# mobvoi/lstm_ctc

Measured on AMD Instinct MI355X. Metric: acoustic frames/sec (whole node), 5xBiLSTM-1024 CTC, higher is better.
Workload: dtype f32

## Files before the change

### lstm_ctc_amd/csrc/common.h

```cpp
#pragma once
#include <hip/hip_runtime.h>
#include <stdint.h>
#include <stdio.h>
#include <stdarg.h>
#include "../../include/lstm_ctc_hip.h"

#define LC_WAVE 64

void lc_set_error(const char *fmt, ...);
enum { LC_OPT_LSTM_PERSISTENT = 0, LC_OPT_LSTM_SPIN_LIMIT, LC_OPT_GEMM_F32_BIG, LC_OPT_GEMM_BF16_BIG, LC_OPT_CTC_LSE2,
       LC_OPT_GEMM_BF16_PERSIST, LC_OPT_GEMM_TAIL };
long lc_option(int opt, long dflt);

#define LC_CHECK_ARG(cond, ...)                                   \
    do {                                                          \
        if (!(cond)) { lc_set_error(__VA_ARGS__); return LC_EINVAL; } \
    } while (0)

#define LC_CHECK_LAUNCH(what)                                                        \
    do {                                                                             \
        hipError_t e_ = hipGetLastError();                                           \
        if (e_ != hipSuccess) {                                                      \
            lc_set_error("%s: %s", what, hipGetErrorString(e_));                     \
            return LC_ELAUNCH;                                                       \
        }                                                                            \
    } while (0)

static inline int lc_cdiv(long long a, long long b) { return (int)((a + b - 1) / b); }

__host__ __device__ inline uint32_t lc_fmix32(uint32_t h)
{
    h ^= h >> 16; h *= 0x85EBCA6Bu; h ^= h >> 13; h *= 0xC2B2AE35u; h ^= h >> 16;
    return h;
}
__host__ __device__ inline float lc_dropout_factor(uint32_t seed, uint32_t stream, uint64_t idx,
                                                   float keep, float inv_keep)
{
    uint32_t h = (seed * 0x9E3779B1u) ^ (stream * 0x85EBCA77u + 0x165667B1u);
    uint32_t v = lc_fmix32((uint32_t)idx ^ h);
    v = lc_fmix32(v ^ ((uint32_t)(idx >> 32) + 0x27D4EB2Fu));
    float u = (float)(v >> 8) * (1.0f / 16777216.0f);
    return u < keep ? inv_keep : 0.0f;
}

__device__ __forceinline__ float lc_wave_shr1(float x, float fill)
{
    return __int_as_float(__builtin_amdgcn_update_dpp(__float_as_int(fill), __float_as_int(x),
                                                      0x138, 0xf, 0xf, false));
}
__device__ __forceinline__ float lc_wave_shl1(float x, float fill)
{
    return __int_as_float(__builtin_amdgcn_update_dpp(__float_as_int(fill), __float_as_int(x),
                                                      0x130, 0xf, 0xf, false));
}
#define LC_DPP_STEP(OP, v, ctrl, rowmask)                                                                   \
    v = OP(v, __int_as_float(__builtin_amdgcn_update_dpp(__float_as_int(v), __float_as_int(v), ctrl, rowmask, \
                                                         0xf, false)))
__device__ __forceinline__ float lc_addf(float a, float b) { return a + b; }
__device__ __forceinline__ float lc_wave_max(float v)
{
    LC_DPP_STEP(fmaxf, v, 0x111, 0xf);
    LC_DPP_STEP(fmaxf, v, 0x112, 0xf);
    LC_DPP_STEP(fmaxf, v, 0x114, 0xf);
    LC_DPP_STEP(fmaxf, v, 0x118, 0xf);
    LC_DPP_STEP(fmaxf, v, 0x142, 0xa);
    LC_DPP_STEP(fmaxf, v, 0x143, 0xc);
    return __int_as_float(__builtin_amdgcn_readlane(__float_as_int(v), 63));
}
__device__ __forceinline__ float lc_wave_sum(float v)
{
#define LC_DPP_ADD(ctrl, rowmask)                                                                            \
    v += __int_as_float(__builtin_amdgcn_update_dpp(0, __float_as_int(v), ctrl, rowmask, 0xf, true))
    LC_DPP_ADD(0x111, 0xf);
    LC_DPP_ADD(0x112, 0xf);
    LC_DPP_ADD(0x114, 0xf);
    LC_DPP_ADD(0x118, 0xf);
    LC_DPP_ADD(0x142, 0xa);
    LC_DPP_ADD(0x143, 0xc);
#undef LC_DPP_ADD
    return __int_as_float(__builtin_amdgcn_readlane(__float_as_int(v), 63));
}
__device__ __forceinline__ float lc_sigmoid(float x)
{
    return __builtin_amdgcn_rcpf(1.0f + __builtin_amdgcn_exp2f(-1.44269504088896341f * x));
}
__device__ __forceinline__ float lc_tanh(float x)
{
    const float t = __builtin_amdgcn_exp2f(-2.88539008177792681f * fabsf(x));
    return copysignf((1.0f - t) * __builtin_amdgcn_rcpf(1.0f + t), x);
}
```

### lstm_ctc_amd/csrc/error.cpp

```cpp
#include <limits.h>
#include <stdarg.h>
#include <stdio.h>
#include <stdlib.h>
#include <string.h>
#include "../../include/lstm_ctc_hip.h"

static thread_local char g_err[512] = "";

void lc_set_error(const char *fmt, ...)
{
    va_list ap;
    va_start(ap, fmt);
    vsnprintf(g_err, sizeof(g_err), fmt, ap);
    va_end(ap);
}

extern "C" const char *lc_last_error(void) { return g_err; }
extern "C" int lc_version(void) { return 2; }

static const char *const g_opt_name[] = {"lstm_persistent", "lstm_spin_limit", "gemm_f32_big", "gemm_bf16_big", "ctc_lse2",
                                         "gemm_bf16_persist", "gemm_tail"};
static const char *const g_opt_env[] = {"LC_LSTM_PERSISTENT", "LC_LSTM_SPIN_LIMIT", "LC_GEMM_F32_BIG",
                                        "LC_GEMM_BF16_BIG", "LC_CTC_LSE2", "LC_GEMM_BF16_PERSIST",
                                        "LC_GEMM_TAIL"};
enum { N_OPTS = sizeof(g_opt_name) / sizeof(g_opt_name[0]) };
static thread_local long g_opt_val[N_OPTS];
static thread_local bool g_opt_set[N_OPTS];

long lc_option(int opt, long dflt)
{
    if (opt < 0 || opt >= N_OPTS) return dflt;
    if (g_opt_set[opt]) return g_opt_val[opt];
    const char *env = getenv(g_opt_env[opt]);
    return env ? atol(env) : dflt;
}
static int opt_index(const char *name)
{
    for (int i = 0; name && i < N_OPTS; ++i)
        if (strcmp(name, g_opt_name[i]) == 0) return i;
    return -1;
}
extern "C" int lc_set_option(const char *name, long value)
{
    const int i = opt_index(name);
    if (i < 0) { lc_set_error("lc_set_option: unknown option '%s'", name ? name : "(null)"); return LC_EINVAL; }
    g_opt_set[i] = value != LC_OPTION_UNSET;
    g_opt_val[i] = value;
    return LC_OK;
}
extern "C" int lc_get_option(const char *name, long *value)
{
    const int i = opt_index(name);
    if (i < 0) { lc_set_error("lc_get_option: unknown option '%s'", name ? name : "(null)"); return LC_EINVAL; }
    const long v = lc_option(i, LC_OPTION_UNSET);
    if (value) *value = v;
    return LC_OK;
}
```

### lstm_ctc_amd/csrc/gemm.hip

```cpp
#include "common.h"
#include "gemm_epi.h"
#include <algorithm>

typedef float f32x16 __attribute__((ext_vector_type(16)));
typedef int i32x4 __attribute__((ext_vector_type(4)));
typedef float f32x4v __attribute__((ext_vector_type(4)));
__device__ f32x4v lc_raw_buffer_load_f32x4(i32x4 rsrc, int voffset, int soffset, int aux) __asm("llvm.amdgcn.raw.buffer.load.v4f32");
__device__ i32x4 lc_raw_buffer_load_i32x4(i32x4 rsrc, int voffset, int soffset, int aux) __asm("llvm.amdgcn.raw.buffer.load.v4i32");

namespace {

#ifndef LC_GEMM_BK
#define LC_GEMM_BK 16
#endif
#ifndef LC_GEMM_GROUP_M
#define LC_GEMM_GROUP_M 8
#endif
constexpr int BM = 128, BN = 128, BK = LC_GEMM_BK, NT = 256;

template <bool KMAJOR, bool FAST, int I>
__device__ __forceinline__ float4 tile_load1(const float *__restrict__ src, int ld, int c0, int cmax, int k0,
                                             int kmax, bool vec_ok)
{
    const int f = threadIdx.x + NT * I;
// ... 705 lines not shown
#pragma unroll
    for (int q = 0; q < 4; ++q) maa[q] = lds0 + arow + so[q];
#define LC_MLOAD(Q, FA, FB)                                                                                            \
    {                                                                                                                  \
        lds_read128<0>(maa[Q] + tbuf, FA[0]); lds_read128<4096>(maa[Q] + tbuf, FA[1]);                                 \
        lds_read128<8192>(maa[Q] + tbuf, FA[2]); lds_read128<12288>(maa[Q] + tbuf, FA[3]);                             \
        _Pragma("unroll") for (int j = 0; j < 2; ++j) tr16_pair<(Q) * 8192>(tob[j] + tbuf, FB[j][0], FB[j][1]);        \
    }
#define LC_MWAIT(FA, FB)                                                                                               \
    asm volatile("s_waitcnt lgkmcnt(0)"                                                                                \
                 : "+v"(FA[0]), "+v"(FA[1]), "+v"(FA[2]), "+v"(FA[3]), "+v"(FB[0][0]), "+v"(FB[0][1]), "+v"(FB[1][0]),  \
                   "+v"(FB[1][1]));
#define LC_MMMA(FA, FB)                                                                                                \
    _Pragma("unroll") for (int i = 0; i < 4; ++i)                                                                      \
        _Pragma("unroll") for (int j = 0; j < 2; ++j)                                                                  \
            acc[i][j] = __builtin_amdgcn_mfma_f32_32x32x16_bf16(frag_cast(FA[i]), tr16_join(FB[j][0], FB[j][1]),        \
                                                               acc[i][j], 0, 0, 0);
#define LC_MCOMPUTE(BUF)                                                                                               \
    {                                                                                                                  \
        const unsigned tbuf = (BUF) * 2 * G_OPERAND_BYTES;                                                             \
        i32x4g m0a[4], m1a[4];                                                                                         \
        i32x2 m0b[2][2], m1b[2][2];                                                                                    \
        LC_MLOAD(0, m0a, m0b) LC_MWAIT(m0a, m0b)                                                                       \
        LC_MLOAD(1, m1a, m1b) LC_MMMA(m0a, m0b) LC_MWAIT(m1a, m1b)                                                     \
        LC_MLOAD(2, m0a, m0b) LC_MMMA(m1a, m1b) LC_MWAIT(m0a, m0b)                                                     \
        LC_MLOAD(3, m1a, m1b) LC_MMMA(m0a, m0b) LC_MWAIT(m1a, m1b)                                                     \
        LC_MMMA(m1a, m1b)                                                                                              \
    }
#define LC_GCOMPUTE(BUF)                                                                                               \
    {                                                                                                                  \
        const unsigned char *as = lds + (BUF) * 2 * G_OPERAND_BYTES;                                                   \
        const unsigned char *bs = lds + ((BUF) * 2 + 1) * G_OPERAND_BYTES;                                             \
        bf16x8 a[4], b[2];                                                                                             \
        _Pragma("unroll") for (int i = 0; i < 4; ++i) a[i] = LC_GFRAG_A(i, 0);                                         \
        _Pragma("unroll") for (int j = 0; j < 2; ++j) b[j] = LC_GFRAG_B(j, 0);                                         \
        _Pragma("unroll") for (int q = 0; q < 4; ++q) {                                                                \
            bf16x8 na[4], nb[2];                                                                                       \
            if (q + 1 < 4) {                                                                                           \
                _Pragma("unroll") for (int i = 0; i < 4; ++i) na[i] = LC_GFRAG_A(i, (q + 1) & 3);                      \
                _Pragma("unroll") for (int j = 0; j < 2; ++j) nb[j] = LC_GFRAG_B(j, (q + 1) & 3);                      \
            }                                                                                                          \
            _Pragma("unroll") for (int i = 0; i < 4; ++i)                                                              \
                _Pragma("unroll") for (int j = 0; j < 2; ++j)                                                          \
                    acc[i][j] = __builtin_amdgcn_mfma_f32_32x32x16_bf16(a[i], b[j], acc[i][j], 0, 0, 0);               \
            if (q + 1 < 4) {                                                                                           \
                _Pragma("unroll") for (int i = 0; i < 4; ++i) a[i] = na[i];                                            \
                _Pragma("unroll") for (int j = 0; j < 2; ++j) b[j] = nb[j];                                            \
            }                                                                                                          \
        }                                                                                                              \
    }
#define LC_GSYNC()                                                                                                     \
    {                                                                                                                  \
        if constexpr (ACOL || BCOL) asm volatile("s_waitcnt vmcnt(0)" ::: "memory");                                   \
        __syncthreads();                                                                                               \
    }
#define LC_GDO(BUF)                                                                                                    \
    {                                                                                                                  \
        if constexpr (ACOL) LC_TCOMPUTE(BUF) else if constexpr (BCOL) LC_MCOMPUTE(BUF) else LC_GCOMPUTE(BUF)            \
    }
    const int ntiles = (p.M / GBM) * (p.N / GBN);
    LC_GFILL(0, 0)
    LC_GSYNC()
    for (int vb = blockIdx.x;;) {
#pragma unroll
    for (int i = 0; i < 4; ++i)
#pragma unroll
        for (int j = 0; j < 2; ++j)
#pragma unroll
            for (int r = 0; r < 16; ++r) acc[i][j][r] = 0.f;
    int nm0 = m0, nn0 = n0;
    bool more = false;
    __amdgpu_buffer_rsrc_t ra_n = ra, rb_n = rb;
    if constexpr (PERSIST) {
        const int vn = vb + (int)gridDim.x;
        more = vn < ntiles;
        if (more) {
            int bm_, bn_;
            gemm_tile_order_big(p.M, p.N, bm_, bn_, vn);
            nm0 = bm_ * GBM; nn0 = bn_ * GBN;
            ra_n = rsrc_a(nm0); rb_n = rsrc_b(nn0);
        }
    }
    int kt = 0;
    for (; kt + 2 <= nk; kt += 2) {
        LC_GFILL(min(kt + 1, nk - 1), 1)
        LC_GDO(0)
        LC_GSYNC()
        if (PERSIST && kt + 2 >= nk) {
            LC_GFILL_FROM(ra_n, rb_n, 0, 0)
        } else {
            LC_GFILL(min(kt + 2, nk - 1), 0)
        }
        LC_GDO(1)
        LC_GSYNC()
    }
    if (kt < nk) LC_GDO(0)
#undef LC_GCOMPUTE
#undef LC_GFRAG
#undef LC_GFRAG_A
#undef LC_GFRAG_B
#undef LC_TLOAD
#undef LC_TWAIT
#undef LC_TMMA
#undef LC_TCOMPUTE
#undef LC_MLOAD
#undef LC_MWAIT
#undef LC_MMMA
#undef LC_MCOMPUTE
    if (p.slab) {
        float *S = p.slab + (size_t)blockIdx.z * p.slab_slice;
#pragma unroll
        for (int i = 0; i < 4; ++i)
#pragma unroll
            for (int j = 0; j < 2; ++j) {
                const int col = n0 + wn * 64 + j * 32 + lr;
#pragma unroll
                for (int r = 0; r < 16; ++r) {
                    const int row = m0 + wm * 128 + i * 32 + (r & 3) + 8 * (r >> 2) + 4 * lk;
                    S[(size_t)row * p.slab_ld + col] = acc[i][j][r];
                }
            }
        return;
    }
#pragma unroll
    for (int i = 0; i < 4; ++i)
#pragma unroll
        for (int j = 0; j < 2; ++j) {
            const int col = n0 + wn * 64 + j * 32 + lr;
            const float bv = p.bias ? p.bias[col] : 0.f;
            unsigned est;
            int ecm;
            epi_column(p.epi, col, est, ecm);
#pragma unroll
            for (int r = 0; r < 16; ++r) {
                const int row = m0 + wm * 128 + i * 32 + (r & 3) + 8 * (r >> 2) + 4 * lk;
                float *c = p.C + (size_t)row * p.ldc + col;
                float v = p.alpha * acc[i][j][r] + bv;
                if (p.beta != 0.f) v += p.beta * *c;
                epi_store(p.epi, c, v, row, col, est, ecm);
            }
        }
    if constexpr (!PERSIST) break;
    if (!more) break;
    vb += (int)gridDim.x;
    m0 = nm0; n0 = nn0; ra = ra_n; rb = rb_n;
    }
#undef LC_GSYNC
#undef LC_GDO
#undef LC_GFILL
#undef LC_GFILL_FROM
}

constexpr int FGBK = 32;
template <bool ACOL, bool BCOL, bool SEG2 = false>
__global__ __launch_bounds__(GNT, 1) void gemm_f32g_kernel(GemmArgs p)
{
    static_assert(!SEG2 || (!ACOL && !BCOL), "two operand pairs: NT form");
    __shared__ __attribute__((aligned(1024))) unsigned char lds[4 * 256 * FGBK * 4];
    constexpr int OPB = 256 * FGBK * 4;
    int bm, bn;
    gemm_tile_order_big(p.M, p.N, bm, bn);
    const int m0 = bm * GBM, n0 = bn * GBN;
    const int lane = threadIdx.x & 63, wave = __builtin_amdgcn_readfirstlane(threadIdx.x >> 6);
    const int wm = wave >> 2, wn = wave & 3;
    const int kbeg = blockIdx.z * p.kchunk;
    const int kend = min(p.K, kbeg + p.kchunk);
    const int nk = (kend - kbeg) / FGBK;
    const float *abase = ACOL ? p.A + (size_t)kbeg * p.lda + m0 : p.A + (size_t)m0 * p.lda + kbeg;
    const float *bbase = BCOL ? p.B + (size_t)kbeg * p.ldb + n0 : p.B + (size_t)n0 * p.ldb + kbeg;
    const __amdgpu_buffer_rsrc_t ra = __builtin_amdgcn_make_buffer_rsrc((void *)abase, 0, 0x7fffffff, 0x00020000);
    const __amdgpu_buffer_rsrc_t rb = __builtin_amdgcn_make_buffer_rsrc((void *)bbase, 0, 0x7fffffff, 0x00020000);
    const int nk1 = SEG2 ? p.k1 / FGBK : nk;
    const __amdgpu_buffer_rsrc_t ra2 = SEG2 ? __builtin_amdgcn_make_buffer_rsrc((void *)(p.A2 + (size_t)m0 * p.lda), 0,
                                                                                0x7fffffff, 0x00020000) : ra;
    const __amdgpu_buffer_rsrc_t rb2 = SEG2 ? __builtin_amdgcn_make_buffer_rsrc((void *)(p.B2 + (size_t)n0 * p.ldb), 0,
                                                                                0x7fffffff, 0x00020000) : rb;
    int voa[4], vob[4];
#pragma unroll
    for (int i = 0; i < 4; ++i) {
        const int piece = wave * 4 + i;
        if (ACOL) voa[i] = (piece * p.lda + 4 * lane) * 4;
        else { const int row = piece * 8 + (lane >> 3); voa[i] = (row * p.lda + ((lane & 7) ^ ((row >> 1) & 7)) * 4) * 4; }
        if (BCOL) vob[i] = (piece * p.ldb + 4 * lane) * 4;
        else { const int row = piece * 8 + (lane >> 3); vob[i] = (row * p.ldb + ((lane & 7) ^ ((row >> 1) & 7)) * 4) * 4; }
    }
    const int ka = ACOL ? FGBK * p.lda * 4 : FGBK * 4, kb = BCOL ? FGBK * p.ldb * 4 : FGBK * 4;
#define LC_FFILL_FROM(RA, RB, KT, BUF)                                                                                 \
    {                                                                                                                  \
        _Pragma("unroll") for (int i = 0; i < 4; ++i)                                                                  \
            __builtin_amdgcn_raw_ptr_buffer_load_lds(RA, lds + (BUF) * 2 * OPB + (wave * 4 + i) * 1024, 16, voa[i],     \
                                                     (KT) * ka, 0, 0);                                                 \
        _Pragma("unroll") for (int i = 0; i < 4; ++i)                                                                  \
            __builtin_amdgcn_raw_ptr_buffer_load_lds(RB, lds + ((BUF) * 2 + 1) * OPB + (wave * 4 + i) * 1024, 16,       \
                                                     vob[i], (KT) * kb, 0, 0);                                         \
    }
#define LC_FFILL(KT, BUF)                                                                                              \
    {                                                                                                                  \
        const int kt_ = (KT);                                                                                          \
        if (SEG2 && kt_ >= nk1) LC_FFILL_FROM(ra2, rb2, kt_ - nk1, BUF) else LC_FFILL_FROM(ra, rb, kt_, BUF)           \
    }
    f32x16 acc[4][2];
#pragma unroll
    for (int i = 0; i < 4; ++i)
#pragma unroll
        for (int j = 0; j < 2; ++j)
#pragma unroll
            for (int r = 0; r < 16; ++r) acc[i][j][r] = 0.f;
    const int lr = lane & 31, lk = lane >> 5;
    const int fl = (lr >> 1) & 7;
    int soq[4];
#pragma unroll
    for (int q = 0; q < 4; ++q) soq[q] = ((2 * q + lk) ^ fl) * 16;
    const int arow = ACOL ? (4 * lk * 256 + wm * 128 + lr) * 4 : (wm * 128 + lr) * 128;
    const int brow = BCOL ? (4 * lk * 256 + wn * 64 + lr) * 4 : (wn * 64 + lr) * 128;
#define LC_FCOMPUTE(BUF)                                                                                               \
    {                                                                                                                  \
        const unsigned char *as = lds + (BUF) * 2 * OPB + arow;                                                        \
        const unsigned char *bs = lds + ((BUF) * 2 + 1) * OPB + brow;                                                  \
        _Pragma("unroll") for (int q = 0; q < 4; ++q) {                                                                \
            float a[4][4], b[2][4];                                                                                    \
            _Pragma("unroll") for (int i = 0; i < 4; ++i) {                                                            \
                if (ACOL) {                                                                                            \
                    _Pragma("unroll") for (int t = 0; t < 4; ++t)                                                      \
                        a[i][t] = *reinterpret_cast<const float *>(as + ((8 * q + t) * 256 + i * 32) * 4);             \
                } else {                                                                                               \
                    const f32x4v v = *reinterpret_cast<const f32x4v *>(as + i * 4096 + soq[q]);                        \
                    a[i][0] = v.x; a[i][1] = v.y; a[i][2] = v.z; a[i][3] = v.w;                                        \
                }                                                                                                      \
            }                                                                                                          \
            _Pragma("unroll") for (int j = 0; j < 2; ++j) {                                                            \
                if (BCOL) {                                                                                            \
                    _Pragma("unroll") for (int t = 0; t < 4; ++t)                                                      \
                        b[j][t] = *reinterpret_cast<const float *>(bs + ((8 * q + t) * 256 + j * 32) * 4);             \
                } else {                                                                                               \
                    const f32x4v v = *reinterpret_cast<const f32x4v *>(bs + j * 4096 + soq[q]);                        \
                    b[j][0] = v.x; b[j][1] = v.y; b[j][2] = v.z; b[j][3] = v.w;                                        \
                }                                                                                                      \
            }                                                                                                          \
            _Pragma("unroll") for (int t = 0; t < 4; ++t)                                                              \
                _Pragma("unroll") for (int i = 0; i < 4; ++i)                                                          \
                    _Pragma("unroll") for (int j = 0; j < 2; ++j)                                                      \
                        acc[i][j] = __builtin_amdgcn_mfma_f32_32x32x2f32(a[i][t], b[j][t], acc[i][j], 0, 0, 0);        \
        }                                                                                                              \
    }
    LC_FFILL(0, 0)
    __syncthreads();
    int kt = 0;
    for (; kt + 2 <= nk; kt += 2) {
        LC_FFILL(min(kt + 1, nk - 1), 1)
        LC_FCOMPUTE(0)
        __syncthreads();
        LC_FFILL(min(kt + 2, nk - 1), 0)
        LC_FCOMPUTE(1)
        __syncthreads();
    }
    if (kt < nk) LC_FCOMPUTE(0)
#undef LC_FFILL
#undef LC_FFILL_FROM
#undef LC_FCOMPUTE
    if (p.slab) {
        float *S = p.slab + (size_t)blockIdx.z * p.slab_slice;
#pragma unroll
        for (int i = 0; i < 4; ++i)
#pragma unroll
            for (int j = 0; j < 2; ++j) {
                const int col = n0 + wn * 64 + j * 32 + lr;
#pragma unroll
                for (int r = 0; r < 16; ++r) {
                    const int row = m0 + wm * 128 + i * 32 + (r & 3) + 8 * (r >> 2) + 4 * lk;
                    S[(size_t)row * p.slab_ld + col] = acc[i][j][r];
                }
            }
        return;
    }
#pragma unroll
    for (int i = 0; i < 4; ++i)
#pragma unroll
        for (int j = 0; j < 2; ++j) {
            const int col = n0 + wn * 64 + j * 32 + lr;
            const float bv = p.bias ? p.bias[col] : 0.f;
            unsigned est;
            int ecm;
            epi_column(p.epi, col, est, ecm);
#pragma unroll
            for (int r = 0; r < 16; ++r) {
                const int row = m0 + wm * 128 + i * 32 + (r & 3) + 8 * (r >> 2) + 4 * lk;
                float *c = p.C + (size_t)row * p.ldc + col;
                float v = p.alpha * acc[i][j][r] + bv;
                if (p.beta != 0.f) v += p.beta * *c;
                epi_store(p.epi, c, v, row, col, est, ecm);
            }
        }
}

__global__ __launch_bounds__(256) void cast_bf16_kernel(const float *__restrict__ x, int rows, int C, int ldx,
                                                        unsigned short *__restrict__ nat, int ldnat,
                                                        unsigned short *__restrict__ tr, int ldtr)
{
    __shared__ unsigned short tile[64][66];
    const int r0 = blockIdx.y * 64, c0 = blockIdx.x * 64;
    const int tx = threadIdx.x & 63, ty = threadIdx.x >> 6;
    for (int i = ty; i < 64; i += 4) {
        const int r = r0 + i, c = c0 + tx;
        unsigned short v = 0;
        if (r < rows && c < C) {
            v = __builtin_bit_cast(unsigned short, (__bf16)x[(size_t)r * ldx + c]);
            if (nat) nat[(size_t)r * ldnat + c] = v;
        }
        tile[i][tx] = v;
    }
    if (!tr) return;
    __syncthreads();
    for (int i = ty; i < 64; i += 4) {
        const int c = c0 + i, r = r0 + tx;
        if (c < C && r < rows) tr[(size_t)c * ldtr + r] = tile[tx][i];
    }
}

__device__ __forceinline__ unsigned cast_pack2(float lo, float hi)
{
    return (unsigned)__builtin_bit_cast(unsigned short, (__bf16)lo) |
           ((unsigned)__builtin_bit_cast(unsigned short, (__bf16)hi) << 16);
}
template <bool NAT, bool TR>
__global__ __launch_bounds__(256) void cast_bf16_vec_kernel(const float *__restrict__ x, int ldx,
                                                            unsigned short *__restrict__ nat, int ldnat,
                                                            unsigned short *__restrict__ tr, int ldtr)
{
    __shared__ __attribute__((aligned(16))) unsigned tile[64 * 32];
    const int r0 = blockIdx.y * 64, c0 = blockIdx.x * 64;
    const int cq = threadIdx.x & 15, rp = threadIdx.x >> 4;
#pragma unroll
    for (int i = 0; i < 2; ++i) {
        const int rpair = rp + 16 * i;
        const size_t r = (size_t)r0 + 2 * rpair;
        const int c = c0 + 4 * cq;
        const float4 v0 = *reinterpret_cast<const float4 *>(x + r * ldx + c);
        const float4 v1 = *reinterpret_cast<const float4 *>(x + (r + 1) * ldx + c);
        if constexpr (NAT) {
            *reinterpret_cast<uint2 *>(nat + r * ldnat + c) = make_uint2(cast_pack2(v0.x, v0.y), cast_pack2(v0.z, v0.w));
            *reinterpret_cast<uint2 *>(nat + (r + 1) * ldnat + c) = make_uint2(cast_pack2(v1.x, v1.y), cast_pack2(v1.z, v1.w));
        }
        if constexpr (TR) {
            const int slot = rpair ^ ((cq & 7) << 2);
            tile[(4 * cq + 0) * 32 + slot] = cast_pack2(v0.x, v1.x);
            tile[(4 * cq + 1) * 32 + slot] = cast_pack2(v0.y, v1.y);
            tile[(4 * cq + 2) * 32 + slot] = cast_pack2(v0.z, v1.z);
            tile[(4 * cq + 3) * 32 + slot] = cast_pack2(v0.w, v1.w);
        }
    }
    if constexpr (TR) {
        __syncthreads();
#pragma unroll
        for (int i = 0; i < 2; ++i) {
            const int c = (threadIdx.x >> 3) + 32 * i, g = threadIdx.x & 7;
            const uint4 v = *reinterpret_cast<const uint4 *>(&tile[c * 32 + ((4 * g) ^ (((c >> 2) & 7) << 2))]);
            *reinterpret_cast<uint4 *>(tr + (size_t)(c0 + c) * ldtr + r0 + 8 * g) = v;
        }
    }
}

__global__ __launch_bounds__(256) void splitk_reduce_kernel(const float *__restrict__ slab, int nslices, int M, int N,
                                                            float alpha, float beta, float *__restrict__ C, int ldc,
                                                            const float *__restrict__ bias)
{
    const size_t total = (size_t)M * N / 4;
    for (size_t i = blockIdx.x * (size_t)blockDim.x + threadIdx.x; i < total; i += (size_t)gridDim.x * blockDim.x) {
        const size_t e = i * 4;
        const int row = (int)(e / N), col = (int)(e % N);
        float4 s = *reinterpret_cast<const float4 *>(slab + e);
        for (int k = 1; k < nslices; ++k) {
            const float4 t = *reinterpret_cast<const float4 *>(slab + (size_t)k * M * N + e);
            s.x += t.x; s.y += t.y; s.z += t.z; s.w += t.w;
        }
        float *c = C + (size_t)row * ldc + col;
        float o[4] = {alpha * s.x, alpha * s.y, alpha * s.z, alpha * s.w};
#pragma unroll
        for (int q = 0; q < 4; ++q) {
            if (bias) o[q] += bias[col + q];
            if (beta != 0.f) o[q] += beta * c[q];
            c[q] = o[q];
        }
    }
}

inline bool aligned16(const void *p) { return (((uintptr_t)p) & 15) == 0; }

inline int pick_splitk(int M, int N, int K)
{
    const long long tiles = (long long)lc_cdiv(M, BM) * lc_cdiv(N, BN);
    if (tiles >= 1536 || K < 4096 || (N % 4) != 0) return 1;
    const long long slots = 768;
    int best = 1;
    double best_eff = 0.0;
    for (int s = 1; s <= 32 && (long long)K / s >= 1024; ++s) {
        const long long wg = tiles * s, rounds = (wg + slots - 1) / slots;
        const double eff = (double)wg / (double)(rounds * slots);
        if (eff > best_eff + 1e-9) { best_eff = eff; best = s; }
    }
    return best;
}

inline int pick_splitk_big(int M, int N, int K, int bk = GBK)
{
    if (M <= 0 || N <= 0 || M % GBM || N % GBN || K < bk || K % bk) return 0;
    const long long tiles = (long long)(M / GBM) * (N / GBN);
    if (tiles >= 512 || K < 4096) return 1;
    int best = 1;
    double best_eff = 0.0;
    for (int c = 1; c <= 32 && K / c >= 1024; ++c) {
        const long long wg = tiles * c, rounds = (wg + 255) / 256;
        const double eff = (double)wg / (double)(rounds * 256);
        if (eff > best_eff + 1e-9) { best_eff = eff; best = c; }
    }
    return best;
}

}

static int lc_num_cus()
{
    static int cached[16] = {0};
    int dev = 0;
    if (hipGetDevice(&dev) != hipSuccess || dev < 0 || dev >= 16) return 256;
    if (cached[dev] == 0) {
        int n = 0;
        if (hipDeviceGetAttribute(&n, hipDeviceAttributeMultiprocessorCount, dev) != hipSuccess || n <= 0) n = 256;
        cached[dev] = n;
    }
    return cached[dev];
}
static int gemm_whole_round_row_tiles(int row_tiles, int col_tiles, int cus_override = 0)
{
    const int cus = cus_override > 0 ? cus_override : lc_num_cus();
    if (lc_option(LC_OPT_GEMM_TAIL, 0) == 0 || row_tiles <= 1 || col_tiles <= 0) return row_tiles;
    const long long tiles = (long long)row_tiles * col_tiles;
    if (tiles % cus == 0 || tiles < 2ll * cus) return row_tiles;
    double best_t = (double)((tiles + cus - 1) / cus) - 0.05;
    int best = row_tiles;
    for (int keep = row_tiles - 1, it = 0; keep >= 1 && it < 512; --keep, ++it) {
        const long long big = (long long)keep * col_tiles, rem = big % cus;
        if (big < cus) break;
        if (rem != 0 && rem * 100 < (long long)cus * 97) continue;
        const double t = (double)((big + cus - 1) / cus) + (double)(row_tiles - keep) * col_tiles * 4 * 0.275 / cus + 0.1;
        if (t < best_t) { best_t = t; best = keep; }
    }
    return best;
}
extern "C" int lc_debug_gemm_whole_round_row_tiles(int row_tiles, int col_tiles, int cus)
{
    return gemm_whole_round_row_tiles(row_tiles, col_tiles, cus);
}
static bool bf16g_persist_ok(long long tiles, int nsl, int K)
{
    const int cus = lc_num_cus();
    return lc_option(LC_OPT_GEMM_BF16_PERSIST, 0) != 0 && nsl <= 1 && K % (2 * GBK) == 0 && cus % 8 == 0 && tiles > cus;
}

static const EpiArgs EPI_NONE = {1.f, 1.f, 0u, 0u, 1, nullptr, 0, 0, 0};
static thread_local EpiArgs g_epi_next = EPI_NONE;
EpiArgs lc_epi_take()
{
    const EpiArgs e = g_epi_next;
    g_epi_next = EPI_NONE;
    return e;
}
static EpiArgs epi_take() { return lc_epi_take(); }
extern "C" int lc_gemm_next_epilogue(const lc_gemm_epilogue_t *e)
{
    if (!e) { g_epi_next = EPI_NONE; return LC_OK; }
    LC_CHECK_ARG(e->keep > 0.f && e->keep <= 1.f && (e->keep >= 1.f || e->drop_width > 0),
                 "lc_gemm_next_epilogue: keep must be in (0, 1] and drop_width > 0");
    LC_CHECK_ARG(!e->c_bf16 || e->ldc_bf16 > 0, "lc_gemm_next_epilogue: ldc_bf16 must be positive");
    EpiArgs a = EPI_NONE;
    a.keep = e->keep; a.inv_keep = 1.0f / e->keep; a.seed = e->seed; a.stream0 = e->stream0;
    a.P = e->keep < 1.f ? e->drop_width : 1;
    a.c16 = (unsigned short *)e->c_bf16; a.ldc16 = e->ldc_bf16;
    LC_CHECK_ARG(!e->shadow_only || e->c_bf16, "lc_gemm_next_epilogue: shadow_only needs c_bf16");
    a.skip_c = e->shadow_only ? 1 : 0;
    g_epi_next = a;
    return LC_OK;
}

extern "C" size_t lc_gemm_workspace_bytes(int M, int N, int K)
{
    const int s = std::max(pick_splitk(M, N, K), std::max(pick_splitk_big(M, N, K), pick_splitk_big(M, N, K, FGBK)));
    return s > 1 ? (size_t)s * M * N * sizeof(float) : 0;
}

static void gemm_launch_part(bool bf16, bool fast, int ta, int tb, GemmArgs p, int nsl, hipStream_t s)
{
    const long long nwg = (long long)lc_cdiv(p.M, BM) * lc_cdiv(p.N, BN);
    dim3 grid((unsigned)nwg, 1, (unsigned)(nsl > 1 ? nsl : 1)), block(NT);
#define LC_GEMM(TA, TB)                                                                          \
    do {                                                                                         \
        if (bf16) {                                                                              \
            if (fast) hipLaunchKernelGGL((gemm_bf16_kernel<TA, TB, true>), grid, block, 0, s, p);    \
            else hipLaunchKernelGGL((gemm_bf16_kernel<TA, TB, false>), grid, block, 0, s, p);        \
        } else {                                                                                 \
            if (fast) hipLaunchKernelGGL((gemm_f32_kernel<TA, TB, true>), grid, block, 0, s, p);     \
            else hipLaunchKernelGGL((gemm_f32_kernel<TA, TB, false>), grid, block, 0, s, p);         \
        }                                                                                        \
    } while (0)
    if (!ta && !tb) LC_GEMM(false, false);
    else if (ta && !tb) LC_GEMM(true, false);
    else if (!ta && tb) LC_GEMM(false, true);
    else LC_GEMM(true, true);
#undef LC_GEMM
}

static int gemm_launch(bool bf16, const char *who, int ta, int tb, int M, int N, int K, float alpha, const float *A,
                       int lda, const float *B, int ldb, float beta, float *C, int ldc, const float *bias,
                       void *workspace, size_t workspace_bytes, lc_stream_t stream)
{
    const EpiArgs epi = epi_take();
    LC_CHECK_ARG(A && B && C, "%s: null pointer", who);
    LC_CHECK_ARG(M >= 0 && N >= 0 && K >= 0, "%s: negative dimension", who);
    if (M == 0 || N == 0) return LC_OK;
    LC_CHECK_ARG(lda >= (ta ? M : K) && ldb >= (tb ? K : N) && ldc >= N, "%s: leading dimension too small", who);
    hipStream_t s = (hipStream_t)stream;
    const int bk = bf16 ? HBK : BK;
    if (epi_active(epi)) { workspace = nullptr; workspace_bytes = 0; }
    GemmArgs p;
    p.epi = epi;
    p.A2 = p.B2 = nullptr; p.k1 = 0;
    p.M = M; p.N = N; p.K = K; p.alpha = alpha; p.beta = beta;
    p.A = A; p.lda = lda; p.B = B; p.ldb = ldb; p.C = C; p.ldc = ldc; p.bias = bias;
    p.vecA = aligned16(A) && (lda % 4 == 0);
    p.vecB = aligned16(B) && (ldb % 4 == 0);
    LC_CHECK_ARG((long long)lc_cdiv(M, BM) * lc_cdiv(N, BN) < (1ll << 31), "%s: grid too large", who);
    const int big_mode = (int)lc_option(LC_OPT_GEMM_F32_BIG, 1);
    if (!bf16 && big_mode != 0 && p.vecA && p.vecB && K >= FGBK && K % FGBK == 0) {
        int Mi = M / GBM * GBM;
        const int Ni = N / GBN * GBN;
        const bool exact = Mi == M && Ni == N;
        int nb = exact ? pick_splitk_big(M, N, K, FGBK) : 1;
        if (nb > 1 && (!workspace || workspace_bytes < (size_t)nb * M * N * sizeof(float))) nb = 1;
        if (nb <= 1) Mi = gemm_whole_round_row_tiles(Mi / GBM, Ni / GBN) * GBM;
        const long long tiles = (long long)(Mi / GBM) * (Ni / GBN);
        const long long spanA = ta ? (long long)K * lda * 4 + 4ll * GBM : (long long)(GBM - 1) * lda * 4 + 4ll * K;
        const long long spanB = tb ? (long long)(GBN - 1) * ldb * 4 + 4ll * K : (long long)K * ldb * 4 + 4ll * GBN;
        const long long wgs = tiles * (nb > 1 ? nb : 1), rounds = (wgs + 255) / 256;
        const bool fills = wgs >= 128 && wgs * 10 >= rounds * 256 * 9;
        if (tiles > 0 && (fills || big_mode == 2) && spanA < 0x7fffffffll && spanB < 0x7fffffffll) {
            GemmArgs q = p;
            q.M = Mi; q.N = Ni;
            q.kchunk = nb > 1 ? lc_cdiv(lc_cdiv(K, nb), FGBK) * FGBK : K;
            if (nb > 1) nb = lc_cdiv(K, q.kchunk);
            q.slab = nb > 1 ? (float *)workspace : nullptr;
            q.slab_slice = (size_t)M * N;
            q.slab_ld = N;
            const dim3 grid((unsigned)tiles, 1, (unsigned)(nb > 1 ? nb : 1)), block(GNT);
            if (ta && !tb) hipLaunchKernelGGL((gemm_f32g_kernel<true, true>), grid, block, 0, s, q);
            else if (ta) hipLaunchKernelGGL((gemm_f32g_kernel<true, false>), grid, block, 0, s, q);
            else if (!tb) hipLaunchKernelGGL((gemm_f32g_kernel<false, true>), grid, block, 0, s, q);
            else hipLaunchKernelGGL((gemm_f32g_kernel<false, false>), grid, block, 0, s, q);
            p.kchunk = K > 0 ? K : 1; p.slab = nullptr; p.slab_slice = 0; p.slab_ld = N;
            if (Ni < N) {
                q = p;
                q.N = N - Ni;
                q.B = tb ? B + (size_t)Ni * ldb : B + Ni;
                q.C = C + Ni;
                q.epi = epi_block(p.epi, 0, Ni);
                q.bias = bias ? bias + Ni : nullptr;
                q.vecB = aligned16(q.B) && (ldb % 4 == 0);
                gemm_launch_part(false, false, ta, tb, q, 1, s);
            }
            if (Mi < M) {
                q = p;
                q.M = M - Mi; q.N = Ni;
                q.A = ta ? A + Mi : A + (size_t)Mi * lda;
                q.C = C + (size_t)Mi * ldc;
                q.epi = epi_block(p.epi, Mi, 0);
                q.vecA = aligned16(q.A) && (lda % 4 == 0);
                const bool fast = q.M % BM == 0 && q.N % BN == 0 && K % BK == 0 && q.vecA && q.vecB;
                gemm_launch_part(false, fast, ta, tb, q, 1, s);
            }
            LC_CHECK_LAUNCH(who);
            if (nb > 1) {
                const size_t quads = (size_t)M * N / 4;
                int g = (int)((quads + 255) / 256);
                if (g > 2048) g = 2048;
                hipLaunchKernelGGL(splitk_reduce_kernel, dim3(g), dim3(256), 0, s, (float *)workspace, nb, M, N, alpha, beta, C, ldc, bias);
                LC_CHECK_LAUNCH("splitk_reduce");
            }
            return LC_OK;
        }
    }
    int nsl = pick_splitk(M, N, K);
    if (nsl > 1 && (!workspace || workspace_bytes < (size_t)nsl * M * N * sizeof(float))) nsl = 1;
    p.kchunk = nsl > 1 ? lc_cdiv(lc_cdiv(K, nsl), bk) * bk : (K > 0 ? K : 1);
    if (nsl > 1) nsl = lc_cdiv(K, p.kchunk);
    p.slab = nsl > 1 ? (float *)workspace : nullptr;
    p.slab_slice = (size_t)M * N;
    p.slab_ld = N;
    const bool kfast = (K % bk == 0) && K > 0 && p.vecA && p.vecB && (p.kchunk % bk == 0);
    const int Mi = M / BM * BM, Ni = N / BN * BN;
    const bool ragged = Mi < M || Ni < N;
    const long long interior_wgs = (long long)(Mi / BM) * (Ni / BN) * (nsl > 1 ? nsl : 1);
    if (kfast && Mi > 0 && Ni > 0 && !(ragged && interior_wgs < 256)) {
        GemmArgs q = p;
        q.M = Mi; q.N = Ni;
        gemm_launch_part(bf16, true, ta, tb, q, nsl, s);
        if (Ni < N) {
            q = p;
            q.N = N - Ni;
            q.B = tb ? B + (size_t)Ni * ldb : B + Ni;
            q.C = C + Ni;
            q.epi = epi_block(p.epi, 0, Ni);
            q.bias = bias ? bias + Ni : nullptr;
            q.vecB = aligned16(q.B) && (ldb % 4 == 0);
            if (q.slab) q.slab += Ni;
            gemm_launch_part(bf16, false, ta, tb, q, nsl, s);
        }
        if (Mi < M) {
            q = p;
            q.M = M - Mi; q.N = Ni;
            q.A = ta ? A + Mi : A + (size_t)Mi * lda;
            q.C = C + (size_t)Mi * ldc;
            q.epi = epi_block(p.epi, Mi, 0);
            q.vecA = aligned16(q.A) && (lda % 4 == 0);
            if (q.slab) q.slab += (size_t)Mi * N;
            gemm_launch_part(bf16, false, ta, tb, q, nsl, s);
        }
    } else {
        gemm_launch_part(bf16, false, ta, tb, p, nsl, s);
    }
    LC_CHECK_LAUNCH(who);
    if (nsl > 1) {
        const size_t quads = (size_t)M * N / 4;
        int g = (int)((quads + 255) / 256);
        if (g > 2048) g = 2048;
        hipLaunchKernelGGL(splitk_reduce_kernel, dim3(g), dim3(256), 0, s, p.slab, nsl, M, N, alpha, beta, C, ldc, bias);
        LC_CHECK_LAUNCH("splitk_reduce");
    }
    return LC_OK;
}

extern "C" int lc_gemm_f32(int ta, int tb, int M, int N, int K, float alpha, const float *A, int lda,
                           const float *B, int ldb, float beta, float *C, int ldc, const float *bias,
                           void *workspace, size_t workspace_bytes, lc_stream_t stream)
{
    return gemm_launch(false, "lc_gemm_f32", ta, tb, M, N, K, alpha, A, lda, B, ldb, beta, C, ldc, bias, workspace,
                       workspace_bytes, stream);
}

extern "C" int lc_gemm_f32_nt2(int M, int N, int K1, int K2, float alpha, const float *A1, const float *A2, int lda,
                               const float *B1, const float *B2, int ldb, float beta, float *C, int ldc, const float *bias,
                               lc_stream_t stream)
{
    const EpiArgs epi = epi_take();
    const char *who = "lc_gemm_f32_nt2";
    LC_CHECK_ARG(A1 && A2 && B1 && B2 && C, "%s: null pointer", who);
    LC_CHECK_ARG(M >= 0 && N >= 0 && K1 > 0 && K2 > 0, "%s: bad dimension", who);
    if (M == 0 || N == 0) return LC_OK;
    LC_CHECK_ARG(lda >= std::max(K1, K2) && ldb >= std::max(K1, K2) && ldc >= N, "%s: leading dimension too small", who);
    hipStream_t s = (hipStream_t)stream;
    auto sequence = [&](int m, int n, const float *a1, const float *a2, const float *b1, const float *b2, float *c,
                        const float *bi, const EpiArgs &e) -> int {
        int rc = gemm_launch(false, who, 0, 1, m, n, K1, alpha, a1, lda, b1, ldb, beta, c, ldc, bi, nullptr, 0, stream);
        if (rc != LC_OK) return rc;
        g_epi_next = e;
        return gemm_launch(false, who, 0, 1, m, n, K2, alpha, a2, lda, b2, ldb, 1.f, c, ldc, nullptr, nullptr, 0, stream);
    };
    const int Mi = M / GBM * GBM, Ni = N / GBN * GBN;
    const long long tiles = (long long)(Mi / GBM) * (Ni / GBN), rounds = (tiles + 255) / 256;
    const int big_mode = (int)lc_option(LC_OPT_GEMM_F32_BIG, 1);
    const bool vec = aligned16(A1) && aligned16(A2) && aligned16(B1) && aligned16(B2) && lda % 4 == 0 && ldb % 4 == 0;
    const bool fills = tiles >= 128 && tiles * 10 >= rounds * 256 * 9;
    const long long span = (long long)(GBM - 1) * std::max(lda, ldb) * 4 + 4ll * std::max(K1, K2);
    if (!(big_mode != 0 && vec && tiles > 0 && (fills || big_mode == 2) && K1 % FGBK == 0 && K2 % FGBK == 0 &&
          span < 0x7fffffffll))
        return sequence(M, N, A1, A2, B1, B2, C, bias, epi);
    GemmArgs q;
    q.epi = epi;
    q.M = Mi; q.N = Ni; q.K = K1 + K2; q.alpha = alpha; q.beta = beta;
    q.A = A1; q.lda = lda; q.B = B1; q.ldb = ldb; q.C = C; q.ldc = ldc; q.bias = bias;
    q.vecA = q.vecB = 1;
    q.kchunk = K1 + K2; q.slab = nullptr; q.slab_slice = 0; q.slab_ld = N;
    q.A2 = A2; q.B2 = B2; q.k1 = K1;
    hipLaunchKernelGGL((gemm_f32g_kernel<false, false, true>), dim3((unsigned)tiles, 1, 1), dim3(GNT), 0, s, q);
    LC_CHECK_LAUNCH(who);
    if (Ni < N) {
        const int rc = sequence(M, N - Ni, A1, A2, B1 + (size_t)Ni * ldb, B2 + (size_t)Ni * ldb, C + Ni,
                                bias ? bias + Ni : nullptr, epi_block(epi, 0, Ni));
        if (rc != LC_OK) return rc;
    }
    if (Mi < M) {
        const int rc = sequence(M - Mi, Ni, A1 + (size_t)Mi * lda, A2 + (size_t)Mi * lda, B1, B2, C + (size_t)Mi * ldc, bias,
                                epi_block(epi, Mi, 0));
        if (rc != LC_OK) return rc;
    }
    return LC_OK;
}
extern "C" int lc_gemm_bf16(int ta, int tb, int M, int N, int K, float alpha, const float *A, int lda,
                            const float *B, int ldb, float beta, float *C, int ldc, const float *bias,
                            void *workspace, size_t workspace_bytes, lc_stream_t stream)
{
    return gemm_launch(true, "lc_gemm_bf16", ta, tb, M, N, K, alpha, A, lda, B, ldb, beta, C, ldc, bias, workspace,
                       workspace_bytes, stream);
}

extern "C" int lc_cast_bf16(const float *x, int rows, int C, int ldx, uint16_t *nat, int ldnat, uint16_t *tr, int ldtr,
                            lc_stream_t stream)
{
    LC_CHECK_ARG(x && (nat || tr) && rows >= 0 && C > 0 && ldx >= C, "lc_cast_bf16: bad argument");
    LC_CHECK_ARG((!nat || ldnat >= C) && (!tr || ldtr >= rows), "lc_cast_bf16: leading dimension too small");
    if (rows == 0) return LC_OK;
    if (rows % 64 == 0 && C % 64 == 0 && ldx % 4 == 0 && aligned16(x) && (!nat || (ldnat % 4 == 0 && (((uintptr_t)nat) & 7) == 0)) &&
        (!tr || (ldtr % 8 == 0 && aligned16(tr)))) {
        const dim3 grid(C / 64, rows / 64), block(256);
        hipStream_t s = (hipStream_t)stream;
        if (nat && tr) hipLaunchKernelGGL((cast_bf16_vec_kernel<true, true>), grid, block, 0, s, x, ldx, nat, ldnat, tr, ldtr);
        else if (nat) hipLaunchKernelGGL((cast_bf16_vec_kernel<true, false>), grid, block, 0, s, x, ldx, nat, ldnat, tr, ldtr);
        else hipLaunchKernelGGL((cast_bf16_vec_kernel<false, true>), grid, block, 0, s, x, ldx, nat, ldnat, tr, ldtr);
        LC_CHECK_LAUNCH("cast_bf16 (64 x 64 tiles)");
        return LC_OK;
    }
    hipLaunchKernelGGL(cast_bf16_kernel, dim3(lc_cdiv(C, 64), lc_cdiv(rows, 64)), dim3(256), 0, (hipStream_t)stream, x, rows,
                       C, ldx, nat, ldnat, tr, ldtr);
    LC_CHECK_LAUNCH("cast_bf16");
    return LC_OK;
}

static int gemm_bf16_nt_impl(const EpiArgs &epi, int M, int N, int K, float alpha, const uint16_t *A, int lda, const uint16_t *B,
                             int ldb, float beta, float *C, int ldc, const float *bias, void *workspace,
                             size_t workspace_bytes, lc_stream_t stream, const uint16_t *A2 = nullptr,
                             const uint16_t *B2 = nullptr, int K2 = 0)
{
    if (epi_active(epi)) { workspace = nullptr; workspace_bytes = 0; }
    LC_CHECK_ARG(A && B && C, "lc_gemm_bf16_nt: null pointer");
    LC_CHECK_ARG(M >= 0 && N >= 0 && K >= 0, "lc_gemm_bf16_nt: negative dimension");
    if (M == 0 || N == 0) return LC_OK;
    LC_CHECK_ARG(lda >= K && ldb >= K && ldc >= N, "lc_gemm_bf16_nt: leading dimension too small");
    LC_CHECK_ARG(K % 8 == 0 && lda % 8 == 0 && ldb % 8 == 0 && aligned16(A) && aligned16(B),
                 "lc_gemm_bf16_nt: K, lda, ldb must be multiples of 8 and the operands 16-byte aligned");
    hipStream_t s = (hipStream_t)stream;
    SGemmArgs sp;
    GemmArgs &p = sp.g;
    p.M = M; p.N = N; p.K = K; p.alpha = alpha; p.beta = beta;
    p.A = nullptr; p.lda = lda; p.B = nullptr; p.ldb = ldb; p.C = C; p.ldc = ldc; p.bias = bias;
    p.vecA = p.vecB = 1;
    p.epi = epi;
    sp.A = A; sp.B = B;
    LC_CHECK_ARG((long long)lc_cdiv(M, BM) * lc_cdiv(N, BN) < (1ll << 31), "lc_gemm_bf16_nt: grid too large");
    sp.A2 = sp.B2 = nullptr; sp.k1 = 0;
    const bool big_off = lc_option(LC_OPT_GEMM_BF16_BIG, 1) == 0;
    int Mb = M / GBM * GBM;
    const int Nb = N / GBN * GBN;
    const bool seg2 = A2 != nullptr;
    if (!seg2 && !(Mb == M && Nb == N && pick_splitk_big(M, N, K) > 1))
        Mb = gemm_whole_round_row_tiles(Mb / GBM, Nb / GBN) * GBM;
    const bool big_ok = !big_off && Mb > 0 && Nb > 0 && K >= GBK && K % GBK == 0 &&
        (long long)(GBM - 1) * lda * 2 + 2ll * std::max(K, K2) < 0x7fffffffll &&
        (long long)(GBN - 1) * ldb * 2 + 2ll * std::max(K, K2) < 0x7fffffffll && (!seg2 || (K2 >= GBK && K2 % GBK == 0));
    if (seg2 && !big_ok) {
        int rc = gemm_bf16_nt_impl(EPI_NONE, M, N, K, alpha, A, lda, B, ldb, beta, C, ldc, bias, workspace, workspace_bytes, stream);
        if (rc != LC_OK) return rc;
        return gemm_bf16_nt_impl(epi, M, N, K2, alpha, A2, lda, B2, ldb, 1.f, C, ldc, nullptr, nullptr, 0, stream);
    }
    if (big_ok) {
        const long long tiles = (long long)(Mb / GBM) * (Nb / GBN);
        int nsl = (Mb == M && Nb == N && !seg2) ? pick_splitk_big(M, N, K) : 1;
        if (nsl > 1 && (!workspace || workspace_bytes < (size_t)nsl * M * N * sizeof(float))) nsl = 1;
        SGemmArgs q = sp;
        q.g.M = Mb; q.g.N = Nb;
        q.g.kchunk = nsl > 1 ? lc_cdiv(lc_cdiv(K, nsl), GBK) * GBK : K;
        if (nsl > 1) nsl = lc_cdiv(K, q.g.kchunk);
        q.g.slab = nsl > 1 ? (float *)workspace : nullptr;
        q.g.slab_slice = (size_t)M * N;
        q.g.slab_ld = N;
        if (seg2) {
            q.A2 = A2; q.B2 = B2; q.k1 = K;
            q.g.K = K + K2; q.g.kchunk = K + K2;
            hipLaunchKernelGGL((gemm_bf16g_kernel<false, false, false, true>), dim3((unsigned)tiles, 1, 1), dim3(GNT), 0, s, q);
        } else if (bf16g_persist_ok(tiles, nsl, K))
            hipLaunchKernelGGL((gemm_bf16g_kernel<false, false, true>), dim3((unsigned)lc_num_cus(), 1, 1), dim3(GNT), 0, s, q);
        else
            hipLaunchKernelGGL((gemm_bf16g_kernel<false, false>), dim3((unsigned)tiles, 1, (unsigned)(nsl > 1 ? nsl : 1)), dim3(GNT), 0, s, q);
        p.kchunk = K; p.slab = nullptr; p.slab_slice = 0; p.slab_ld = N;
        auto strip = [&](const SGemmArgs &r0) {
            const long long nwg = (long long)lc_cdiv(r0.g.M, BM) * lc_cdiv(r0.g.N, BN);
            if (!seg2) {
                if (r0.g.M % BM == 0 && r0.g.N % BN == 0 && K % SBK == 0)
                    hipLaunchKernelGGL((gemm_bf16s_kernel<true>), dim3((unsigned)nwg, 1, 1), dim3(NT), 0, s, r0);
                else
                    hipLaunchKernelGGL((gemm_bf16s_kernel<false>), dim3((unsigned)nwg, 1, 1), dim3(NT), 0, s, r0);
                return;
            }
            SGemmArgs r = r0;
            const EpiArgs e = r.g.epi;
            r.g.epi = EPI_NONE;
            hipLaunchKernelGGL((gemm_bf16s_kernel<false>), dim3((unsigned)nwg, 1, 1), dim3(NT), 0, s, r);
            r.A = A2 + (r0.A - A); r.B = B2 + (r0.B - B);
            r.g.K = K2; r.g.kchunk = K2; r.g.beta = 1.f; r.g.bias = nullptr; r.g.epi = e;
            hipLaunchKernelGGL((gemm_bf16s_kernel<false>), dim3((unsigned)nwg, 1, 1), dim3(NT), 0, s, r);
        };
        if (Nb < N) {
            q = sp;
            q.g.N = N - Nb;
            q.B = B + (size_t)Nb * ldb;
            q.g.C = C + Nb;
            q.g.epi = epi_block(p.epi, 0, Nb);
            q.g.bias = bias ? bias + Nb : nullptr;
            strip(q);
        }
        if (Mb < M) {
            q = sp;
            q.g.M = M - Mb; q.g.N = Nb;
            q.A = A + (size_t)Mb * lda;
            q.g.C = C + (size_t)Mb * ldc;
            q.g.epi = epi_block(p.epi, Mb, 0);
            strip(q);
        }
        LC_CHECK_LAUNCH("lc_gemm_bf16_nt (256 x 256 tiles)");
        if (nsl > 1) {
            const size_t quads = (size_t)M * N / 4;
            int g = (int)((quads + 255) / 256);
            if (g > 2048) g = 2048;
            hipLaunchKernelGGL(splitk_reduce_kernel, dim3(g), dim3(256), 0, s, (float *)workspace, nsl, M, N, alpha, beta, C, ldc, bias);
            LC_CHECK_LAUNCH("splitk_reduce");
        }
        return LC_OK;
    }
    int nsl = pick_splitk(M, N, K);
    if (nsl > 1 && (!workspace || workspace_bytes < (size_t)nsl * M * N * sizeof(float))) nsl = 1;
    p.kchunk = nsl > 1 ? lc_cdiv(lc_cdiv(K, nsl), SBK) * SBK : (K > 0 ? K : 1);
    if (nsl > 1) nsl = lc_cdiv(K, p.kchunk);
    p.slab = nsl > 1 ? (float *)workspace : nullptr;
    p.slab_slice = (size_t)M * N;
    p.slab_ld = N;
    auto launch = [&](bool fast, const SGemmArgs &q) {
        const long long nwg = (long long)lc_cdiv(q.g.M, BM) * lc_cdiv(q.g.N, BN);
        dim3 grid((unsigned)nwg, 1, (unsigned)(nsl > 1 ? nsl : 1)), block(NT);
// ... 127 lines not shown
```

Measured before the change: 187,100.

## Software-pipeline LDS fragment reads against MFMA in f32 GEMM k-loop

Adds a templated k-loop schedule to the f32 MFMA GEMM kernel. Fragments for the next k-step are read from LDS while the current step's MFMAs issue, using double-buffered register fragments and sched_barriers to fix the order. Mode 2 also prefetches two LDS tiles and places the global fill and barrier in the middle of the compute. Mode 2 is the default only for the !ACOL && BCOL variant, selectable via a new option. This raises register pressure and adds scheduling complexity; vmcnt(0) waits may stall.

```diff
diff --git a/lstm_ctc_amd/csrc/common.h b/lstm_ctc_amd/csrc/common.h
--- a/lstm_ctc_amd/csrc/common.h
+++ b/lstm_ctc_amd/csrc/common.h
@@ -9,7 +9,7 @@
 
 void lc_set_error(const char *fmt, ...);
 enum { LC_OPT_LSTM_PERSISTENT = 0, LC_OPT_LSTM_SPIN_LIMIT, LC_OPT_GEMM_F32_BIG, LC_OPT_GEMM_BF16_BIG, LC_OPT_CTC_LSE2,
-       LC_OPT_GEMM_BF16_PERSIST, LC_OPT_GEMM_TAIL };
+       LC_OPT_GEMM_BF16_PERSIST, LC_OPT_GEMM_TAIL, LC_OPT_GEMM_F32_PIPE };
 long lc_option(int opt, long dflt);
 
 #define LC_CHECK_ARG(cond, ...)                                   \
diff --git a/lstm_ctc_amd/csrc/error.cpp b/lstm_ctc_amd/csrc/error.cpp
--- a/lstm_ctc_amd/csrc/error.cpp
+++ b/lstm_ctc_amd/csrc/error.cpp
@@ -19,10 +19,10 @@
 extern "C" int lc_version(void) { return 2; }
 
 static const char *const g_opt_name[] = {"lstm_persistent", "lstm_spin_limit", "gemm_f32_big", "gemm_bf16_big", "ctc_lse2",
-                                         "gemm_bf16_persist", "gemm_tail"};
+                                         "gemm_bf16_persist", "gemm_tail", "gemm_f32_pipe"};
 static const char *const g_opt_env[] = {"LC_LSTM_PERSISTENT", "LC_LSTM_SPIN_LIMIT", "LC_GEMM_F32_BIG",
                                         "LC_GEMM_BF16_BIG", "LC_CTC_LSE2", "LC_GEMM_BF16_PERSIST",
-                                        "LC_GEMM_TAIL"};
+                                        "LC_GEMM_TAIL", "LC_GEMM_F32_PIPE"};
 enum { N_OPTS = sizeof(g_opt_name) / sizeof(g_opt_name[0]) };
 static thread_local long g_opt_val[N_OPTS];
 static thread_local bool g_opt_set[N_OPTS];
diff --git a/lstm_ctc_amd/csrc/gemm.hip b/lstm_ctc_amd/csrc/gemm.hip
--- a/lstm_ctc_amd/csrc/gemm.hip
+++ b/lstm_ctc_amd/csrc/gemm.hip
@@ -881,10 +881,11 @@
 }
 
 constexpr int FGBK = 32;
-template <bool ACOL, bool BCOL, bool SEG2 = false>
+template <bool ACOL, bool BCOL, bool SEG2 = false, int PIPE = 0>
 __global__ __launch_bounds__(GNT, 1) void gemm_f32g_kernel(GemmArgs p)
 {
     static_assert(!SEG2 || (!ACOL && !BCOL), "two operand pairs: NT form");
+    static_assert(PIPE >= 0 && PIPE <= 2, "k-loop schedule");
     __shared__ __attribute__((aligned(1024))) unsigned char lds[4 * 256 * FGBK * 4];
     constexpr int OPB = 256 * FGBK * 4;
     int bm, bn;
@@ -972,21 +973,114 @@
                         acc[i][j] = __builtin_amdgcn_mfma_f32_32x32x2f32(a[i][t], b[j][t], acc[i][j], 0, 0, 0);        \
         }                                                                                                              \
     }
-    LC_FFILL(0, 0)
-    __syncthreads();
-    int kt = 0;
-    for (; kt + 2 <= nk; kt += 2) {
-        LC_FFILL(min(kt + 1, nk - 1), 1)
-        LC_FCOMPUTE(0)
+    float fa[2][4][4], fb[2][2][4];
+#define LC_FREAD_A(S, AS, Q, H, I)                                                                                     \
+    {                                                                                                                  \
+        if (ACOL) {                                                                                                    \
+            _Pragma("unroll") for (int t_ = 2 * (H); t_ < 2 * (H) + 2; ++t_)                                           \
+                fa[S][I][t_] = *reinterpret_cast<const float *>((AS) + ((8 * (Q) + t_) * 256 + (I) * 32) * 4);         \
+        } else if ((H) == 0) {                                                                                         \
+            const f32x4v v = *reinterpret_cast<const f32x4v *>((AS) + (I) * 4096 + soq[Q]);                            \
+            fa[S][I][0] = v.x; fa[S][I][1] = v.y; fa[S][I][2] = v.z; fa[S][I][3] = v.w;                                \
+        }                                                                                                              \
+    }
+#define LC_FREAD_B(S, BS, Q, H, J)                                                                                     \
+    {                                                                                                                  \
+        if (BCOL) {                                                                                                    \
+            _Pragma("unroll") for (int t_ = 2 * (H); t_ < 2 * (H) + 2; ++t_)                                           \
+                fb[S][J][t_] = *reinterpret_cast<const float *>((BS) + ((8 * (Q) + t_) * 256 + (J) * 32) * 4);         \
+        } else if ((H) == 0) {                                                                                         \
+            const f32x4v v = *reinterpret_cast<const f32x4v *>((BS) + (J) * 4096 + soq[Q]);                            \
+            fb[S][J][0] = v.x; fb[S][J][1] = v.y; fb[S][J][2] = v.z; fb[S][J][3] = v.w;                                \
+        }                                                                                                              \
+    }
+#define LC_FREAD_ALL(S, AS, BS, Q)                                                                                     \
+    {                                                                                                                  \
+        _Pragma("unroll") for (int h = 0; h < 2; ++h) {                                                                \
+            _Pragma("unroll") for (int i = 0; i < 4; ++i) LC_FREAD_A(S, AS, Q, h, i)                                   \
+            _Pragma("unroll") for (int j = 0; j < 2; ++j) LC_FREAD_B(S, BS, Q, h, j)                                   \
+        }                                                                                                              \
+        __builtin_amdgcn_sched_barrier(0);                                                                             \
+    }
+#define LC_FGROUP(S, PRE, AS, BS, Q)                                                                                   \
+    {                                                                                                                  \
+        _Pragma("unroll") for (int t = 0; t < 4; ++t)                                                                  \
+            _Pragma("unroll") for (int i = 0; i < 4; ++i)                                                              \
+                _Pragma("unroll") for (int j = 0; j < 2; ++j) {                                                        \
+                    if ((PRE) && t < 2 && (j == 0 || i < 2)) {                                                         \
+                        if (j == 0) LC_FREAD_A((S) ^ 1, AS, Q, t, i) else LC_FREAD_B((S) ^ 1, BS, Q, t, i)             \
+                        __builtin_amdgcn_sched_barrier(0);                                                             \
+                    }                                                                                                  \
+                    acc[i][j] = __builtin_amdgcn_mfma_f32_32x32x2f32(fa[S][i][t], fb[S][j][t], acc[i][j], 0, 0, 0);    \
+                }                                                                                                      \
+        __builtin_amdgcn_sched_barrier(0);                                                                             \
+    }
+#define LC_FSYNC()                                                                                                     \
+    {                                                                                                                  \
+        asm volatile("s_waitcnt vmcnt(0)" ::: "memory");                                                               \
+        __syncthreads();                                                                                               \
+        __builtin_amdgcn_sched_barrier(0);                                                                             \
+    }
+#define LC_FCOMPUTE1(BUF)                                                                                              \
+    {                                                                                                                  \
+        const unsigned char *as = lds + (BUF) * 2 * OPB + arow;                                                        \
+        const unsigned char *bs = lds + ((BUF) * 2 + 1) * OPB + brow;                                                  \
+        LC_FREAD_ALL(0, as, bs, 0)                                                                                     \
+        LC_FGROUP(0, true, as, bs, 1) LC_FGROUP(1, true, as, bs, 2) LC_FGROUP(0, true, as, bs, 3)                      \
+        LC_FGROUP(1, false, as, bs, 0)                                                                                 \
+    }
+#define LC_FTILE2(BUF, KT)                                                                                             \
+    {                                                                                                                  \
+        const unsigned char *as = lds + (BUF) * 2 * OPB + arow;                                                        \
+        const unsigned char *bs = lds + ((BUF) * 2 + 1) * OPB + brow;                                                  \
+        const unsigned char *an = lds + ((BUF) ^ 1) * 2 * OPB + arow;                                                  \
+        const unsigned char *bn = lds + (((BUF) ^ 1) * 2 + 1) * OPB + brow;                                            \
+        const int kn_ = (KT) + 2;                                                                                      \
+        LC_FGROUP(0, true, as, bs, 1) LC_FGROUP(1, true, as, bs, 2) LC_FGROUP(0, true, as, bs, 3)                      \
+        LC_FSYNC()                                         \
+        if (kn_ < nk) LC_FFILL(kn_, BUF)                                                                               \
+        LC_FGROUP(1, true, an, bn, 0)                                                                                  \
+    }
+    if constexpr (PIPE == 2) {
+        LC_FFILL(0, 0)
+        if (nk > 1) LC_FFILL(1, 1)
+        LC_FSYNC()
+        LC_FREAD_ALL(0, lds + arow, lds + OPB + brow, 0)
+        int kt = 0;
+        for (; kt + 2 < nk; kt += 2) {
+            LC_FTILE2(0, kt)
+            LC_FTILE2(1, kt + 1)
+        }
+        if (kt + 2 == nk) LC_FTILE2(0, kt)
+        const unsigned char *as = lds + ((nk - 1) & 1) * 2 * OPB + arow, *bs = lds + ((nk - 1) & 1) * 2 * OPB + OPB + brow;
+        LC_FGROUP(0, true, as, bs, 1) LC_FGROUP(1, true, as, bs, 2) LC_FGROUP(0, true, as, bs, 3)
+        LC_FGROUP(1, false, as, bs, 0)
+    } else {
+        LC_FFILL(0, 0)
         __syncthreads();
-        LC_FFILL(min(kt + 2, nk - 1), 0)
-        LC_FCOMPUTE(1)
-        __syncthreads();
-    }
-    if (kt < nk) LC_FCOMPUTE(0)
+        int kt = 0;
+        for (; kt + 2 <= nk; kt += 2) {
+            LC_FFILL(min(kt + 1, nk - 1), 1)
+            if constexpr (PIPE == 1) LC_FCOMPUTE1(0) else LC_FCOMPUTE(0)
+            __syncthreads();
+            LC_FFILL(min(kt + 2, nk - 1), 0)
+            if constexpr (PIPE == 1) LC_FCOMPUTE1(1) else LC_FCOMPUTE(1)
+            __syncthreads();
+        }
+        if (kt < nk) {
+            if constexpr (PIPE == 1) LC_FCOMPUTE1(0) else LC_FCOMPUTE(0)
+        }
+    }
 #undef LC_FFILL
 #undef LC_FFILL_FROM
 #undef LC_FCOMPUTE
+#undef LC_FCOMPUTE1
+#undef LC_FTILE2
+#undef LC_FSYNC
+#undef LC_FGROUP
+#undef LC_FREAD_ALL
+#undef LC_FREAD_A
+#undef LC_FREAD_B
     if (p.slab) {
         float *S = p.slab + (size_t)blockIdx.z * p.slab_slice;
 #pragma unroll
@@ -1145,6 +1239,15 @@
     return best;
 }
 
+}
+
+template <bool ACOL, bool BCOL, bool SEG2>
+static void gemm_f32g_launch(dim3 grid, dim3 block, hipStream_t s, const GemmArgs &q)
+{
+    const long pipe = lc_option(LC_OPT_GEMM_F32_PIPE, (!ACOL && BCOL) ? 2 : 0);
+    if (pipe <= 0) hipLaunchKernelGGL((gemm_f32g_kernel<ACOL, BCOL, SEG2, 0>), grid, block, 0, s, q);
+    else if (pipe == 1) hipLaunchKernelGGL((gemm_f32g_kernel<ACOL, BCOL, SEG2, 1>), grid, block, 0, s, q);
+    else hipLaunchKernelGGL((gemm_f32g_kernel<ACOL, BCOL, SEG2, 2>), grid, block, 0, s, q);
 }
 
 static int lc_num_cus()
@@ -1280,10 +1383,10 @@
             q.slab_slice = (size_t)M * N;
             q.slab_ld = N;
             const dim3 grid((unsigned)tiles, 1, (unsigned)(nb > 1 ? nb : 1)), block(GNT);
-            if (ta && !tb) hipLaunchKernelGGL((gemm_f32g_kernel<true, true>), grid, block, 0, s, q);
-            else if (ta) hipLaunchKernelGGL((gemm_f32g_kernel<true, false>), grid, block, 0, s, q);
-            else if (!tb) hipLaunchKernelGGL((gemm_f32g_kernel<false, true>), grid, block, 0, s, q);
-            else hipLaunchKernelGGL((gemm_f32g_kernel<false, false>), grid, block, 0, s, q);
+            if (ta && !tb) gemm_f32g_launch<true, true, false>(grid, block, s, q);
+            else if (ta) gemm_f32g_launch<true, false, false>(grid, block, s, q);
+            else if (!tb) gemm_f32g_launch<false, true, false>(grid, block, s, q);
+            else gemm_f32g_launch<false, false, false>(grid, block, s, q);
             p.kchunk = K > 0 ? K : 1; p.slab = nullptr; p.slab_slice = 0; p.slab_ld = N;
             if (Ni < N) {
                 q = p;
@@ -1408,7 +1511,7 @@
     q.vecA = q.vecB = 1;
     q.kchunk = K1 + K2; q.slab = nullptr; q.slab_slice = 0; q.slab_ld = N;
     q.A2 = A2; q.B2 = B2; q.k1 = K1;
-    hipLaunchKernelGGL((gemm_f32g_kernel<false, false, true>), dim3((unsigned)tiles, 1, 1), dim3(GNT), 0, s, q);
+    gemm_f32g_launch<false, false, true>(dim3((unsigned)tiles, 1, 1), dim3(GNT), s, q);
     LC_CHECK_LAUNCH(who);
     if (Ni < N) {
         const int rc = sequence(M, N - Ni, A1, A2, B1 + (size_t)Ni * ldb, B2 + (size_t)Ni * ldb, C + Ni,
```

New measurement: 187,200, median of 4. About the same (+0.0%).
